# gmarcais/Jellyfish

Measured on AMD Instinct MI355X. Metric: k-mers/sec at k=21 canonical, 150 bp synthetic reads, bit-exact counts, higher is better.
Workload: dtype u64

## Files before the change

### jellyfish_amd/csrc/jfgpu.hip

```cpp
#include <hip/hip_runtime.h>
#include <math.h>
#include <stdint.h>
#include <stdio.h>
#include <string.h>
#include <algorithm>
#include <chrono>
#include <memory>
#include <string>
#include <type_traits>
#include <vector>

#include "../../include/jfgpu.h"
#include "gf2_matrix.hpp"
#include "tuning.hpp"
#include "kernels.hip.hpp"
#include "kernels_part.hip.hpp"
#include "kernels_tile.hip.hpp"
#include "kernels_p1ring.hip.hpp"
#include "kernels_bloom.hip.hpp"
#include "kernels_bloom_part.hip.hpp"
#include "kernels_wide.hip.hpp"
#include "kernels_wide_part.hip.hpp"
#include "kernels_nword.hip.hpp"
#include "kernels_parse.hip.hpp"
// ... 569 lines not shown
  if(!t->part_ok || t->mode == MODE_DIRECT) return false;
  if(t->mode == MODE_PARTITIONED) return true;
  return nbytes >= kPartMinBytes || !t->pending.empty();
}

}

extern "C" {

const char* jfgpu_last_error(void) { return g_err.c_str(); }
int jfgpu_abi_version(void) { return JFGPU_ABI_VERSION; }

int jfgpu_device_count(void) {
  int n = 0;
  if(hipGetDeviceCount(&n) != hipSuccess) return 0;
  return n;
}

int jfgpu_create(const jfgpu_params* p, jfgpu_table** out) {
  if(!p || !out) return fail(JFGPU_E_INVALID, "null argument");
  *out = nullptr;
  if(p->k < 1) return fail(JFGPU_E_INVALID, "mer length must be >= 1");
  if(p->k > 128) return fail(JFGPU_E_UNSUPPORTED, "mer length > 128 (more than four key words) is not built");
  if(p->shard_bits > 8) return fail(JFGPU_E_INVALID, "at most 256 shards");
  if(p->shard_id >= (1u << p->shard_bits)) return fail(JFGPU_E_INVALID, "shard_id out of range");
  int ndev = 0;
  if(hipGetDeviceCount(&ndev) != hipSuccess || ndev == 0)
    return fail(JFGPU_E_NO_DEVICE, "no HIP device: the engine has no CPU fallback");
  int dev = p->device;
  if(dev < 0) HIP_TRY(hipGetDevice(&dev));
  if(dev >= ndev) return fail(JFGPU_E_NO_DEVICE, "device ordinal out of range");
  HIP_TRY(hipSetDevice(dev));

  const bool nword = p->k > 64, wide = p->k > 32 && !nword;
  uint32_t lsize = 0;
  while(lsize < 63 && (1ull << lsize) < p->size) ++lsize;
  if(nword) {
    lsize = std::max(lsize, nword_min_lsize(p->k));
    lsize = std::max<uint32_t>(lsize, kNTileBits + p->shard_bits);
    lsize = std::min<uint32_t>(lsize, 48);
  } else if(wide) {
    lsize = std::max(lsize, wide_min_lsize(p->k));
    lsize = std::max<uint32_t>(lsize, kMaxTileBits + p->shard_bits);
    lsize = std::min<uint32_t>(lsize, 48);
  } else {
    lsize = std::max(lsize, geom_min_lsize(p->k, p->shard_bits));
    lsize = std::max(lsize, p->shard_bits);
    lsize = std::max<uint32_t>(lsize, 1);
    lsize = std::min<uint32_t>(lsize, 2 * p->k);
    if(lsize < p->shard_bits) return fail(JFGPU_E_INVALID, "more shards than 4^k table positions");
  }

  std::unique_ptr<jfgpu_table> t(new jfgpu_table);
  t->tun = Tuning::from_env();
  t->tun.p2_cap = t->tun.p2_cap / kGran * kGran;
  t->params = *p; t->params.matrix_columns = nullptr;
  t->device = dev;
  t->out_counter_len = p->out_counter_len ? p->out_counter_len : 4;
  if(t->out_counter_len > 8) return fail(JFGPU_E_INVALID, "out_counter_len must be <= 8");
  t->wide = wide; t->nword = nword; t->key_words = (2 * p->k + 63) / 64; t->slot_words = nword ? kNWords : wide ? 2 : 1;
  if(nword) {
    if(!nword_geom_init(t->nt.N, p->k, lsize, p->canonical ? 1 : 0, p->shard_bits, p->shard_id)) return fail(JFGPU_E_INVALID, "table geometry does not fit a 256-bit slot");
    t->g = t->nt.N.g;
  } else if(wide) {
    if(!wide_geom_init(t->wt.W, p->k, lsize, p->canonical ? 1 : 0, p->shard_bits, p->shard_id)) return fail(JFGPU_E_INVALID, "table geometry does not fit a 128-bit slot");
    t->g = t->wt.W.g;
  } else if(!geom_init(t->g, p->k, lsize, p->shard_bits, p->shard_id, p->canonical ? 1 : 0, !t->tun.slot64))
    return fail(JFGPU_E_INVALID, "table geometry does not fit a 64-bit slot");

  if(p->matrix_columns) {
    t->matrix.r = lsize; t->matrix.c = 2 * p->k;
    t->matrix.columns.assign(p->matrix_columns, p->matrix_columns + 2 * p->k);
    t->matrix.identity = gf2_is_low_identity(t->matrix);
  } else if(p->matrix_seed) {
    t->matrix = gf2_random(lsize, 2 * p->k, p->matrix_seed);
  } else if(p->k <= 64 && lsize < 2 * p->k && (p->matrix_kind ? p->matrix_kind : (uint32_t)t->tun.matrix) == JFGPU_MATRIX_XORSHIFT) {
    t->xs_matrix = true;
    t->matrix = gf2_xorshift_matrix(lsize, 2 * p->k);
  } else {
    t->ref_matrix = true;
    t->matrix = lsize >= 2 * p->k ? gf2_identity(lsize, 2 * p->k) : gf2_reference_matrix(lsize, 2 * p->k, t->glibc);
  }
  if(!nword) {
    t->g.hash_xs = gf2_is_xorshift(t->matrix) ? 1 : 0;
    if(wide) t->wt.W.g.hash_xs = t->g.hash_xs;
  }
  std::vector<uint64_t> fwd, inv;
  while(!gf2_build_tables(t->matrix, fwd, inv)) {
    if(!t->ref_matrix || t->matrix.identity) return fail(JFGPU_E_INVALID, "hash matrix: low r x r block is singular");
    t->matrix = gf2_reference_matrix(lsize, 2 * p->k, t->glibc);
  }

  hipDeviceProp_t prop;
  HIP_TRY(hipGetDeviceProperties(&prop, dev));
  t->n_cu = prop.multiProcessorCount > 0 ? prop.multiProcessorCount : 256;
  HIP_TRY(hipStreamCreateWithFlags(&t->stream, hipStreamNonBlocking));

  const uint64_t n_slots = 1ull << t->g.lsize_l;
  t->ovf_cap = std::max<uint64_t>(kMinOvf, std::min<uint64_t>(n_slots / 256, 1ull << 26));
  { uint64_t c = 1; while(c < t->ovf_cap) c <<= 1; t->ovf_cap = c; }
  t->returning = t->g.cnt_bits < 40;

  DevTable& d = t->dt;
  d.g = t->g;
  HIP_TRY(hipMalloc((void**)&d.slots, n_slots * slot_bytes_of(t.get())));
  HIP_TRY(hipMalloc((void**)&t->d_fwd, fwd.size() * sizeof(uint64_t)));
  HIP_TRY(hipMalloc((void**)&t->d_inv, inv.size() * sizeof(uint64_t)));
  HIP_TRY(hipMalloc((void**)&d.ovf_key, t->ovf_cap * sizeof(uint64_t)));
  HIP_TRY(hipMalloc((void**)&d.ovf_cnt, t->ovf_cap * sizeof(uint64_t)));
  HIP_TRY(hipMalloc((void**)&d.counters, CTR_COUNT * sizeof(uint64_t)));
  HIP_TRY(hipMalloc((void**)&d.dirty, (size_t)1 << (t->g.lsize_l - t->g.tile_bits)));
  d.fwd_tbl = t->d_fwd; d.inv_tbl = t->d_inv; d.ovf_mask = t->ovf_cap - 1;
  d.max_probe = (uint32_t)std::min<uint64_t>(t->g.tile_mask, 1023);
  HIP_TRY(hipMemcpy(t->d_fwd, fwd.data(), fwd.size() * sizeof(uint64_t), hipMemcpyHostToDevice));
  HIP_TRY(hipMemcpy(t->d_inv, inv.data(), inv.size() * sizeof(uint64_t), hipMemcpyHostToDevice));
  const size_t dump_lds = ((size_t)8 << t->g.tile_bits) + ((size_t)2 << t->g.tile_bits) + (size_t)t->g.nbytes * 2048;
  HIP_TRY(hipFuncSetAttribute((const void*)dump_tiles_kernel, hipFuncAttributeMaxDynamicSharedMemorySize, (int)dump_lds));
  if(nword) {
    NTable& w = t->nt;
    w.slots = d.slots; w.fwd_tbl = d.fwd_tbl; w.inv_tbl = d.inv_tbl; w.ovf_key = d.ovf_key; w.ovf_cnt = d.ovf_cnt;
    w.ovf_mask = d.ovf_mask; w.counters = d.counters; w.max_probe = d.max_probe;
    t->part_ok = false; t->mode = MODE_DIRECT;
    const int nl = (int)(((size_t)32 << kNTileBits) + ((size_t)2 << kNTileBits));
    HIP_TRY(hipFuncSetAttribute((const void*)dump_tiles_words_kernel<NTable>, hipFuncAttributeMaxDynamicSharedMemorySize, nl));
    {
      const int rl = (int)route_lds_bytes(t->g.nbytes, KeyOps<NTable>::kHaloWords);
      HIP_TRY(hipFuncSetAttribute((const void*)route_count_kernel<NTable, false>, hipFuncAttributeMaxDynamicSharedMemorySize, rl));
      HIP_TRY(hipFuncSetAttribute((const void*)route_scatter_kernel<NTable, false>, hipFuncAttributeMaxDynamicSharedMemorySize, rl));
    }
    HIP_TRY(hipFuncSetAttribute((const void*)query_ascii_kernel<NTable>, hipFuncAttributeMaxDynamicSharedMemorySize,
                                (int)query_lds_bytes(t->g.nbytes, KeyOps<NTable>::kHaloWords)));
  } else if(wide) {
    WideTable& w = t->wt;
    w.slots = d.slots; w.fwd_tbl = d.fwd_tbl; w.inv_tbl = d.inv_tbl; w.ovf_key = d.ovf_key; w.ovf_cnt = d.ovf_cnt;
    w.ovf_mask = d.ovf_mask; w.counters = d.counters; w.max_probe = d.max_probe; w.dirty = d.dirty;
    memset(&w.bloom, 0, sizeof w.bloom);
    part_geom_init(t.get());
    const int wl = (int)(((size_t)16 << t->g.tile_bits) + ((size_t)2 << t->g.tile_bits));
    HIP_TRY(hipFuncSetAttribute((const void*)dump_tiles_words_kernel<WideTable>, hipFuncAttributeMaxDynamicSharedMemorySize, wl));
  } else part_geom_init(t.get());
  if(!nword) {
    if(t->tun.mode == 1) t->mode = MODE_DIRECT;
    else if(t->tun.mode == 2 && t->part_ok) t->mode = MODE_PARTITIONED;
  }
  {
#define TATTR2(I, R, S, P, H, M, HL) HIP_TRY(hipFuncSetAttribute((const void*)tile_rank_insert_kernel<I, R, S, P, kTileBlock, H, M, HL>, hipFuncAttributeMaxDynamicSharedMemorySize, (int)tile_rank_lds(sizeof(S), kMaxTileBits, P)))
#define TATTR1(I, R, S, P, H, M) TATTR2(I, R, S, P, H, M, true)
#define TATTR(I, S, P) TATTR1(I, true, S, P, false, false); TATTR1(I, false, S, P, false, false); TATTR1(I, true, S, P, true, false); TATTR1(I, false, S, P, true, false); \
                       TATTR1(I, true, S, P, false, true); TATTR1(I, false, S, P, false, true)
    TATTR(uint32_t, unsigned int, 1); TATTR(uint32_t, unsigned int, 2); TATTR(uint32_t, unsigned long long, 1);
    TATTR(uint64_t, unsigned int, 1); TATTR(uint64_t, unsigned int, 2); TATTR(uint64_t, unsigned long long, 1);
    TATTR2(uint32_t, true, unsigned int, 2, false, false, false); TATTR2(uint32_t, false, unsigned int, 2, false, false, false);
    TATTR2(uint32_t, true, unsigned int, 2, false, true, false); TATTR2(uint32_t, false, unsigned int, 2, false, true, false);
#undef TATTR
#undef TATTR1
#undef TATTR2
    HIP_TRY(hipFuncSetAttribute((const void*)p1_scatter_sorted_kernel<true, true>, hipFuncAttributeMaxDynamicSharedMemorySize, kPTilePos * 6));
    HIP_TRY(hipFuncSetAttribute((const void*)p1_scatter_sorted_kernel<true, false>, hipFuncAttributeMaxDynamicSharedMemorySize, kPTilePos * 6));
    HIP_TRY(hipFuncSetAttribute((const void*)p1_scatter_sorted_kernel<false, true>, hipFuncAttributeMaxDynamicSharedMemorySize, kPTilePos * 6));
    HIP_TRY(hipFuncSetAttribute((const void*)p1_scatter_sorted_kernel<false, false>, hipFuncAttributeMaxDynamicSharedMemorySize, kPTilePos * 6));
#define PATTR(N) HIP_TRY(hipFuncSetAttribute((const void*)p1_keys_scatter_sorted_kernel<N>, hipFuncAttributeMaxDynamicSharedMemorySize, kPTilePos * 6)); \
                 HIP_TRY(hipFuncSetAttribute((const void*)p1_scatter_sorted_kernel<false, false, N>, hipFuncAttributeMaxDynamicSharedMemorySize, kPTilePos * 6))
    PATTR(0); PATTR(6); PATTR(7); PATTR(8);
#undef PATTR
    HIP_TRY(hipFuncSetAttribute((const void*)p1_keys_granule_kernel<true, 0>, hipFuncAttributeMaxDynamicSharedMemorySize, kPTilePos * 6));
    HIP_TRY(hipFuncSetAttribute((const void*)p1_keys_granule_kernel<false, 0>, hipFuncAttributeMaxDynamicSharedMemorySize, kPTilePos * 6));
    HIP_TRY(hipFuncSetAttribute((const void*)p1_keys_granule_kernel<false, 6>, hipFuncAttributeMaxDynamicSharedMemorySize, kPTilePos * 6));
    HIP_TRY(hipFuncSetAttribute((const void*)p1_keys_granule_kernel<false, 7>, hipFuncAttributeMaxDynamicSharedMemorySize, kPTilePos * 6));
    HIP_TRY(hipFuncSetAttribute((const void*)p1_keys_granule_kernel<false, 8>, hipFuncAttributeMaxDynamicSharedMemorySize, kPTilePos * 6));
    {
      const int rl = kGranMaxB * 128 + 128;
#define RATTR(IT, BL, N, CN) HIP_TRY(hipFuncSetAttribute((const void*)p1_ring_kernel<IT, BL, N, CN>, hipFuncAttributeMaxDynamicSharedMemorySize, rl))
      HIP_TRY(hipFuncSetAttribute((const void*)p2_ring_kernel<P2RingDirect>, hipFuncAttributeMaxDynamicSharedMemorySize, rl));
      HIP_TRY(hipFuncSetAttribute((const void*)p2_ring_roles_kernel<uint32_t, 2, P2RingDirect, 1>, hipFuncAttributeMaxDynamicSharedMemorySize, rl));
      HIP_TRY(hipFuncSetAttribute((const void*)p2_ring_roles_kernel<uint32_t, 1, P2RingDirect, 1>, hipFuncAttributeMaxDynamicSharedMemorySize, rl));
      HIP_TRY(hipFuncSetAttribute((const void*)p2_ring_roles_kernel<uint32_t, 2, P2RingDirect, 2>, hipFuncAttributeMaxDynamicSharedMemorySize, rl));
      HIP_TRY(hipFuncSetAttribute((const void*)p2_ring_roles_kernel<uint32_t, 1, P2RingDirect, 2>, hipFuncAttributeMaxDynamicSharedMemorySize, rl));
      HIP_TRY(hipFuncSetAttribute((const void*)p2_ring_roles_kernel<uint32_t, 2, P2RingDirect, 3>, hipFuncAttributeMaxDynamicSharedMemorySize, rl));
      HIP_TRY(hipFuncSetAttribute((const void*)p2_ring_roles_kernel<uint32_t, 1, P2RingDirect, 3>, hipFuncAttributeMaxDynamicSharedMemorySize, rl));
      RATTR(uint32_t, false, 6, 1); RATTR(uint32_t, false, 6, 0); RATTR(uint32_t, true, 0, 2); RATTR(uint32_t, false, 0, 2);
      RATTR(uint32_t, false, kHashXS, 1); RATTR(uint32_t, false, kHashXS, 0); RATTR(uint32_t, false, kHashXSLow, 2);
#undef RATTR
    }
    HIP_TRY(hipFuncSetAttribute((const void*)p2_scatter_sorted_kernel<uint32_t, 16>, hipFuncAttributeMaxDynamicSharedMemorySize, kPBlock * 16 * 4));
    HIP_TRY(hipFuncSetAttribute((const void*)p1_ring_kernel<uint32_t, false, 6, 1, RouteListDirect>, hipFuncAttributeMaxDynamicSharedMemorySize, (int)(kGranMaxB * 128 + 128)));
    HIP_TRY(hipFuncSetAttribute((const void*)p1_ring_kernel<uint32_t, false, 6, 0, RouteListDirect>, hipFuncAttributeMaxDynamicSharedMemorySize, (int)(kGranMaxB * 128 + 128)));
    HIP_TRY(hipFuncSetAttribute((const void*)p1_ring_kernel<uint32_t, false, 0, 2, RouteListDirect>, hipFuncAttributeMaxDynamicSharedMemorySize, (int)(kGranMaxB * 128 + 128)));
    HIP_TRY(hipFuncSetAttribute((const void*)p1_ring_kernel<uint32_t, true, 0, 2, RouteListDirect>, hipFuncAttributeMaxDynamicSharedMemorySize, (int)(kGranMaxB * 128 + 128)));
    HIP_TRY(hipFuncSetAttribute((const void*)p1_ring_kernel<uint32_t, false, kHashXS, 1, RouteListDirect>, hipFuncAttributeMaxDynamicSharedMemorySize, (int)(kGranMaxB * 128 + 128)));
    HIP_TRY(hipFuncSetAttribute((const void*)p1_ring_kernel<uint32_t, false, kHashXS, 0, RouteListDirect>, hipFuncAttributeMaxDynamicSharedMemorySize, (int)(kGranMaxB * 128 + 128)));
    HIP_TRY(hipFuncSetAttribute((const void*)p1_ring_kernel<uint32_t, false, kHashXSLow, 2, RouteListDirect>, hipFuncAttributeMaxDynamicSharedMemorySize, (int)(kGranMaxB * 128 + 128)));
#define SATTR(SW) HIP_TRY(hipFuncSetAttribute((const void*)p2_granule_kernel<uint32_t, TableDirect<true>, kP2PairPer, SW>, hipFuncAttributeMaxDynamicSharedMemorySize, kPBlock * kP2PairPer * 4)); \
                  HIP_TRY(hipFuncSetAttribute((const void*)p2_granule_kernel<uint32_t, TableDirect<false>, kP2PairPer, SW>, hipFuncAttributeMaxDynamicSharedMemorySize, kPBlock * kP2PairPer * 4))
    SATTR(1); SATTR(2); SATTR(4);
#undef SATTR
    HIP_TRY(hipFuncSetAttribute((const void*)p2_granule_kernel<uint64_t, TableDirect<true>, kP2MidPer>, hipFuncAttributeMaxDynamicSharedMemorySize, kPBlock * kP2MidPer * 8));
    HIP_TRY(hipFuncSetAttribute((const void*)p2_granule_kernel<uint64_t, TableDirect<false>, kP2MidPer>, hipFuncAttributeMaxDynamicSharedMemorySize, kPBlock * kP2MidPer * 8));
    HIP_TRY(hipFuncSetAttribute((const void*)p2_granule_kernel<uint32_t, TableDirect<true>, kP2PairPer>, hipFuncAttributeMaxDynamicSharedMemorySize, kPBlock * kP2PairPer * 4));
    HIP_TRY(hipFuncSetAttribute((const void*)p2_granule_kernel<uint32_t, TableDirect<false>, kP2PairPer>, hipFuncAttributeMaxDynamicSharedMemorySize, kPBlock * kP2PairPer * 4));
    HIP_TRY(hipFuncSetAttribute((const void*)p2_scatter_sorted_kernel<uint32_t, kP2PairPer>, hipFuncAttributeMaxDynamicSharedMemorySize, kPBlock * kP2PairPer * 4));
    HIP_TRY(hipFuncSetAttribute((const void*)p2_scatter_sorted_kernel<uint64_t, 14>, hipFuncAttributeMaxDynamicSharedMemorySize, kPBlock * 14 * 8));
    const int gl = kG64Chunk * 10;
    HIP_TRY(hipFuncSetAttribute((const void*)p1_granule64_kernel<true, true, 0>, hipFuncAttributeMaxDynamicSharedMemorySize, gl));
    HIP_TRY(hipFuncSetAttribute((const void*)p1_granule64_kernel<false, true, 0>, hipFuncAttributeMaxDynamicSharedMemorySize, gl));
    HIP_TRY(hipFuncSetAttribute((const void*)p1_granule64_kernel<true, false, 0>, hipFuncAttributeMaxDynamicSharedMemorySize, gl));
    HIP_TRY(hipFuncSetAttribute((const void*)p1_granule64_kernel<false, false, 0>, hipFuncAttributeMaxDynamicSharedMemorySize, gl));
    HIP_TRY(hipFuncSetAttribute((const void*)p1_granule64_kernel<false, false, 7>, hipFuncAttributeMaxDynamicSharedMemorySize, gl));
    HIP_TRY(hipFuncSetAttribute((const void*)p1_granule64_kernel<false, false, 8>, hipFuncAttributeMaxDynamicSharedMemorySize, gl));
    HIP_TRY(hipFuncSetAttribute((const void*)p1_granule64_kernel<false, false, kHashXS>, hipFuncAttributeMaxDynamicSharedMemorySize, gl));
    HIP_TRY(hipFuncSetAttribute((const void*)p1_granule64_kernel<true, false, kHashXS>, hipFuncAttributeMaxDynamicSharedMemorySize, gl));
    HIP_TRY(hipFuncSetAttribute((const void*)p2_granule_kernel<u128, WideDirect<true>, kP2WidePer>, hipFuncAttributeMaxDynamicSharedMemorySize, kPBlock * kP2WidePer * 16));
    HIP_TRY(hipFuncSetAttribute((const void*)p2_granule_kernel<u128, WideDirect<false>, kP2WidePer>, hipFuncAttributeMaxDynamicSharedMemorySize, kPBlock * kP2WidePer * 16));
    HIP_TRY(hipFuncSetAttribute((const void*)p2_scatter_sorted_kernel<u128, 7>, hipFuncAttributeMaxDynamicSharedMemorySize, kPBlock * 7 * 16));
    const int wl = kWideChunk * 18 + 16 * 2048, wt = 16 << kMaxTileBits;
    HIP_TRY(hipFuncSetAttribute((const void*)p1_wide_granule_kernel<true, true>, hipFuncAttributeMaxDynamicSharedMemorySize, wl));
    HIP_TRY(hipFuncSetAttribute((const void*)p1_wide_granule_kernel<true, false>, hipFuncAttributeMaxDynamicSharedMemorySize, wl));
    HIP_TRY(hipFuncSetAttribute((const void*)p1_wide_granule_kernel<false, true>, hipFuncAttributeMaxDynamicSharedMemorySize, wl));
    HIP_TRY(hipFuncSetAttribute((const void*)p1_wide_granule_kernel<false, false>, hipFuncAttributeMaxDynamicSharedMemorySize, wl));
    HIP_TRY(hipFuncSetAttribute((const void*)p1_wide_granule_kernel<true, false, true>, hipFuncAttributeMaxDynamicSharedMemorySize, wl));
    HIP_TRY(hipFuncSetAttribute((const void*)p1_wide_granule_kernel<false, false, true>, hipFuncAttributeMaxDynamicSharedMemorySize, wl));
    HIP_TRY(hipFuncSetAttribute((const void*)tile_insert_wide_kernel<true>, hipFuncAttributeMaxDynamicSharedMemorySize, wt));
    HIP_TRY(hipFuncSetAttribute((const void*)tile_insert_wide_kernel<false>, hipFuncAttributeMaxDynamicSharedMemorySize, wt));
    HIP_TRY(hipFuncSetAttribute((const void*)tile_insert_wide_pipe_kernel<true>, hipFuncAttributeMaxDynamicSharedMemorySize, wt));
    HIP_TRY(hipFuncSetAttribute((const void*)tile_insert_wide_pipe_kernel<false>, hipFuncAttributeMaxDynamicSharedMemorySize, wt));
  }
  jfgpu_table* raw = t.release();
  int rc = jfgpu_clear(raw);
  if(rc) { jfgpu_destroy(raw); return rc; }
  *out = raw;
  return JFGPU_OK;
}

void jfgpu_destroy(jfgpu_table* t) {
  if(!t) return;
  hipSetDevice(t->device);
  if(t->stream) hipStreamSynchronize(t->stream);
  prof_collect(t);
  for(auto e : t->ev_pool) hipEventDestroy(e);
  hipFree(t->dt.slots); hipFree(t->d_fwd); hipFree(t->d_inv);
  if(t->d_dt) hipFree(t->d_dt);
  hipFree(t->dt.ovf_key); hipFree(t->dt.ovf_cnt); hipFree(t->dt.counters); hipFree(t->dt.dirty);
  for(int i = 0; i < 2; ++i) { if(t->d_stage[i]) hipFree(t->d_stage[i]); if(t->stage_done[i]) hipEventDestroy(t->stage_done[i]); }
  if(t->d_dump) hipFree(t->d_dump);
  if(t->d_bcache) hipFree(t->d_bcache);
  if(t->d_tile_off) hipFree(t->d_tile_off);
  part_discard(t);
  if(t->d_M1) hipFree(t->d_M1);
  if(t->d_strag) hipFree(t->d_strag);
  if(t->d_strag2) hipFree(t->d_strag2);
  if(t->d_strag2_n) hipFree(t->d_strag2_n);
  if(t->d_strag_n) hipFree(t->d_strag_n);
  if(t->d_M2) hipFree(t->d_M2);
  if(t->ws) hipFree(t->ws);
  if(t->stream2) hipStreamDestroy(t->stream2);
  for(auto ev : t->flush_ev) if(ev) hipEventDestroy(ev);
  if(t->flush_done) hipEventDestroy(t->flush_done);
  if(t->stream) hipStreamDestroy(t->stream);
  delete t;
}

int jfgpu_get_info(const jfgpu_table* t, jfgpu_info* o) {
  if(!t || !o) return fail(JFGPU_E_INVALID, "null argument");
  memset(o, 0, sizeof(*o));
  o->k = t->g.k; o->key_len = t->g.key_bits; o->canonical = t->g.canonical;
  o->lsize = t->g.lsize_g; o->size = 1ull << t->g.lsize_g; o->local_size = 1ull << t->g.lsize_l;
  o->shard_bits = t->g.shard_bits; o->shard_id = t->g.shard_id;
  o->val_len = t->g.cnt_bits; o->slot_bytes = (uint32_t)slot_bytes_of(t); o->tile_slots = 1u << t->g.tile_bits;
  o->matrix_identity = t->matrix.identity ? 1 : 0;
  o->out_counter_len = t->out_counter_len;
  o->max_reprobe = t->dt.max_probe;
  o->table_bytes = (1ull << t->g.lsize_l) * slot_bytes_of(t);
  return JFGPU_OK;
}

int jfgpu_get_matrix(const jfgpu_table* t, uint64_t* columns) {
  if(!t || !columns) return fail(JFGPU_E_INVALID, "null argument");
  memcpy(columns, t->matrix.columns.data(), sizeof(uint64_t) * t->matrix.c);
  return JFGPU_OK;
}

int jfgpu_clear(jfgpu_table* t) {
  if(t) { t->failed = 0; t->failed_msg.clear(); }
  int rc = use(t); if(rc) return rc;
  part_discard(t);
  HIP_TRY(hipMemsetAsync(t->dt.slots, 0, (1ull << t->g.lsize_l) * slot_bytes_of(t), t->stream));
  HIP_TRY(hipMemsetAsync(t->dt.ovf_key, 0, t->ovf_cap * sizeof(uint64_t), t->stream));
  HIP_TRY(hipMemsetAsync(t->dt.ovf_cnt, 0, t->ovf_cap * sizeof(uint64_t), t->stream));
  HIP_TRY(hipMemsetAsync(t->dt.counters, 0, CTR_COUNT * sizeof(uint64_t), t->stream));
  HIP_TRY(hipMemsetAsync(t->dt.dirty, 0, (size_t)1 << (t->g.lsize_l - t->g.tile_bits), t->stream));
  HIP_TRY(hipStreamSynchronize(t->stream));
  t->pristine = true; t->occ_known = 0; t->fed_since = 0; t->direct_seen = 0; t->occ_bound = 0; t->bigval_bound = 0; t->ovf_failed_need = 0;
  t->flushes_plain = 0; t->flushes_heavy = 0;
  t->n_p2_roles = t->n_p2_ring = t->n_p2_sort = t->n_p2_exact = t->n_p1_ring = t->n_p1_other = t->n_tile_dense = 0;
  return JFGPU_OK;
}

int jfgpu_sync(jfgpu_table* t) {
  int rc = use(t); if(rc) return rc;
  rc = part_flush(t); if(rc) return rc;
  HIP_TRY(hipStreamSynchronize(t->stream));
#ifdef JFGPU_PHASE_PROF
  { unsigned long long c[24], z[24] = {0};
    if(hipMemcpyFromSymbol(c, HIP_SYMBOL(g_phase_prof), sizeof c) == hipSuccess) {
      fprintf(stderr, "[phase prof] P1 (ring): stage %llu  encode+hash+append %llu  (barrier) %llu  units out %llu  finish %llu\n",
              c[0], c[1], c[2], c[3], c[4]);
      fprintf(stderr, "[phase prof] P2: (barrier) %llu  load %llu  hist %llu  scan %llu  lds-scatter %llu  write-out %llu  finish %llu\n",
// ... 552 lines not shown
```

### jellyfish_amd/csrc/kernels_tile.hip.hpp

```cpp
#pragma once
#include "kernels_part.hip.hpp"

namespace jfgpu {

__device__ __attribute__((noinline)) void ovf_add_call(uint64_t* ovf_key, uint64_t* ovf_cnt, uint64_t ovf_mask, uint64_t* counters,
                                                       uint64_t slot, uint64_t units) {
  DevTable V; V.ovf_key = ovf_key; V.ovf_cnt = ovf_cnt; V.ovf_mask = ovf_mask; V.counters = counters;
  ovf_add(V, slot, units);
}

__device__ __forceinline__ uint32_t wg_uniform(uint32_t v) {
#if defined(__HIP_DEVICE_COMPILE__) && !defined(JFGPU_EMU)
  return (uint32_t)__builtin_amdgcn_readfirstlane((int)v);
#else
  return v;
#endif
}

__device__ __forceinline__ void lds_wait_all() {
#if defined(__HIP_DEVICE_COMPILE__) && !defined(JFGPU_EMU)
  __builtin_amdgcn_s_waitcnt(0xC07F);
#endif
}

#ifndef JFGPU_T_BLOCK
#define JFGPU_T_BLOCK 512
#endif
constexpr int kTileBlock = JFGPU_T_BLOCK;
constexpr uint32_t kQueueLook = 2;
#ifndef JFGPU_T_QUEUE
#define JFGPU_T_QUEUE 6144
#endif
constexpr uint32_t kTileQueueBytes = JFGPU_T_QUEUE;

constexpr size_t tile_rank_hdr(size_t nslots) { return (nslots >> kBucketBits) * 2 + 16; }
inline size_t tile_rank_lds(size_t slot_bytes, uint32_t tile_bits, int tpb) {
  const size_t nslots = (size_t)tpb << tile_bits;
  return tile_rank_hdr(nslots) + nslots * slot_bytes + kTileQueueBytes;
}

template <typename ITEM, bool RETURNING, typename SLOT, int TPB, int BLOCK = kTileBlock, bool HEAVY = false, bool SAMPLE = false, bool HOLES = true>
__global__ __launch_bounds__(BLOCK, (BLOCK >= 512 ? 2 * BLOCK / 256 : 4)) void tile_rank_insert_kernel(DevTable T, SegList S, uint64_t tile0, uint32_t n_tiles) {
  constexpr int NP = ((sizeof(ITEM) == 8 || (BLOCK < 512 && TPB == 1)) ? 4608 : 9216) / BLOCK;
  constexpr uint32_t kVec = 16 / sizeof(SLOT);
  constexpr uint32_t kB = 1u << kBucketBits;
  constexpr uint32_t kBV = kB / kVec;
  constexpr uint32_t kSlotBits = 8 * sizeof(SLOT);
  JF_DYN_LDS(s_raw);
  const TableGeom& g = T.g;
  constexpr uint32_t tsz = 1u << kMaxTileBits, nslots = TPB * tsz, nbkt = nslots >> kBucketBits, tmask = tsz - 1;
  constexpr uint32_t NBK = nbkt / BLOCK;
  static_assert(HOLES || (!HEAVY && sizeof(ITEM) == 4), "the hole-free instantiation is the plain kernel's, for 4-byte items");
  constexpr uint32_t kHdr = (uint32_t)tile_rank_hdr(nslots);
  uint32_t* const s_cnt = reinterpret_cast<uint32_t*>(s_raw);
  SLOT* const s_tile = reinterpret_cast<SLOT*>(s_raw + kHdr);
  constexpr uint32_t qcap = kTileQueueBytes / sizeof(ITEM) / (BLOCK / 64);
  static_assert(qcap >= 64, "phase C stages one held-back item per lane through the queue");
  ITEM* const s_q = reinterpret_cast<ITEM*>(s_raw + kHdr + (size_t)nslots * sizeof(SLOT)) + (threadIdx.x >> 6) * qcap;
  SLOT* const gslots = reinterpret_cast<SLOT*>(T.slots);
  const SLOT lmask = (SLOT)g.low_mask, inc = (SLOT)g.inc, occ = (SLOT)g.occ_bit;
  const uint32_t cshift = g.tag_bits + 1, idshift = kSlotBits - cshift;
  const uint32_t lane = threadIdx.x & 63;
  const unsigned long long below = lane ? (~0ull >> (64 - lane)) : 0ull;
  const ITEM hole = (ITEM)~(ITEM)0;

  auto unit_dirty = [&](uint32_t t) -> uint32_t {
    if(TPB == 2) return *reinterpret_cast<const uint16_t*>(T.dirty + tile0 + 2 * (uint64_t)t);
    return T.dirty[tile0 + t];
  };
  auto zero_counters = [&]() {
    for(uint32_t i = threadIdx.x; i < (nbkt >> 1); i += BLOCK) s_cnt[i] = 0;
  };
  auto zero_tile = [&]() {
    for(uint32_t i = threadIdx.x * kVec; i < nslots; i += BLOCK * kVec) *reinterpret_cast<uint4*>(s_tile + i) = make_uint4(0, 0, 0, 0);
  };
  auto load_tile = [&](const SLOT* gt, uint32_t d) {
    for(uint32_t b = threadIdx.x; b < nbkt; b += BLOCK) {
      const bool ld = (d >> (8 * ((b << kBucketBits) >> kMaxTileBits))) & 0xFFu;
      uint32_t c = 0;
#pragma unroll
      for(uint32_t q = 0; q < kBV; ++q) {
        uint4 v = make_uint4(0, 0, 0, 0);
        if(ld) v = *reinterpret_cast<const uint4*>(gt + ((size_t)b << kBucketBits) + q * kVec);
        *reinterpret_cast<uint4*>(s_tile + ((size_t)b << kBucketBits) + q * kVec) = v;
        if(sizeof(SLOT) == 4) c += (v.x != 0) + (v.y != 0) + (v.z != 0) + (v.w != 0);
        else c += ((v.x | v.y) != 0) + ((v.z | v.w) != 0);
      }
      reinterpret_cast<uint16_t*>(s_cnt)[b] = (uint16_t)c;
    }
  };
  auto home_of = [&](ITEM x) -> uint32_t {
    if constexpr(sizeof(ITEM) == 4) return ((uint32_t)x >> g.rem_bits) & (nslots - 1);
    else return (uint32_t)((uint64_t)x >> g.rem_bits) & (nslots - 1);
  };
  auto load_bucket = [&](uint32_t bs, SLOT (&w)[kB]) {
#pragma unroll
    for(uint32_t q = 0; q < kBV; ++q) {
      const uint4 v = *reinterpret_cast<const uint4*>(s_tile + bs + q * kVec);
      if constexpr(sizeof(SLOT) == 4) { w[4 * q] = (SLOT)v.x; w[4 * q + 1] = (SLOT)v.y; w[4 * q + 2] = (SLOT)v.z; w[4 * q + 3] = (SLOT)v.w; }
      else { w[2 * q] = (SLOT)(((uint64_t)v.y << 32) | v.x); w[2 * q + 1] = (SLOT)(((uint64_t)v.w << 32) | v.z); }
    }
  };
  auto store_bucket = [&](uint32_t bs, const SLOT (&w)[kB]) {
#pragma unroll
    for(uint32_t q = 0; q < kBV; ++q) {
      uint4 v;
      if constexpr(sizeof(SLOT) == 4) v = make_uint4((uint32_t)w[4 * q], (uint32_t)w[4 * q + 1], (uint32_t)w[4 * q + 2], (uint32_t)w[4 * q + 3]);
      else v = make_uint4((uint32_t)w[2 * q], (uint32_t)((uint64_t)w[2 * q] >> 32), (uint32_t)w[2 * q + 1], (uint32_t)((uint64_t)w[2 * q + 1] >> 32));
      *reinterpret_cast<uint4*>(s_tile + bs + q * kVec) = v;
    }
  };
  auto has_dups = [&](const SLOT (&w)[kB]) -> bool {
    SLOT sh[kB];
#pragma unroll
    for(uint32_t i = 0; i < kB; ++i) sh[i] = w[i] << idshift;
    bool d = false;
#pragma unroll
    for(uint32_t j = 1; j < kB; ++j) {
      bool e = false;
#pragma unroll
      for(uint32_t i = 0; i < j; ++i) e = e | (sh[i] == sh[j]);
      d = d | (e & (w[j] != 0));
    }
    return d;
  };
  auto merge_bucket = [&](SLOT (&w)[kB], uint64_t bucket_slot0) {
    const SLOT cmask = (SLOT)g.cnt_max;
    SLOT carry[kB];
#pragma unroll
    for(uint32_t i = 0; i < kB; ++i) carry[i] = 0;
#pragma unroll
    for(uint32_t j = 1; j < kB; ++j)
#pragma unroll
      for(uint32_t i = 0; i < j; ++i) {
        const bool same = (w[j] != 0) & (w[i] != 0) & (((w[i] ^ w[j]) & lmask) == 0);
        const SLOT sum = (SLOT)(w[i] >> cshift) + (same ? (SLOT)(w[j] >> cshift) : (SLOT)0);
        w[i] = (w[i] & lmask) | (SLOT)((sum & cmask) << cshift);
        carry[i] += (SLOT)(sum >> g.cnt_bits);
        w[j] = same ? (SLOT)0 : w[j];
      }
    SLOT o[kB], oc[kB];
#pragma unroll
    for(uint32_t i = 0; i < kB; ++i) { o[i] = 0; oc[i] = 0; }
    uint32_t n = 0;
#pragma unroll
    for(uint32_t j = 0; j < kB; ++j) {
      const bool ne = w[j] != 0;
#pragma unroll
      for(uint32_t d = 0; d <= j; ++d) { const bool here = ne & (n == d); o[d] = here ? w[j] : o[d]; oc[d] = here ? carry[j] : oc[d]; }
      n += ne ? 1u : 0u;
    }
    SLOT any = 0;
#pragma unroll
    for(uint32_t q = 0; q < kB; ++q) { w[q] = o[q]; any |= oc[q]; }
    if(RETURNING && any != 0) {
#pragma unroll
      for(uint32_t q = 0; q < kB; ++q) if(oc[q]) ovf_add_call(T.ovf_key, T.ovf_cnt, T.ovf_mask, T.counters, bucket_slot0 + q, (uint64_t)oc[q]);
    }
  };
  auto merge_tile = [&](uint64_t unit_slot0) {
    constexpr uint32_t MB0 = (TPB == 2 && sizeof(ITEM) + sizeof(SLOT) == 8 && NBK >= 4) ? 4 : (NBK >= 2 ? 2 : 1);
    constexpr uint32_t Rmax = nbkt / (BLOCK / 64);
    static_assert(Rmax >= 128, "the merge list must fit the bucket counters");
    constexpr uint32_t R = Rmax >= 512 ? 512 : Rmax >= 256 ? 256 : 128;
    constexpr uint32_t MBr = R >= 512 ? 4 : R >= 256 ? 2 : 1;
    constexpr uint32_t MBw = 16 / kB >= 1 ? 16 / kB : 1;
    constexpr uint32_t MB = MB0 < MBr ? (MB0 < MBw ? MB0 : MBw) : (MBr < MBw ? MBr : MBw);
    static_assert((BLOCK / 64) * R * 2 <= nbkt * 2, "the merge list must fit the bucket counters");
    uint16_t* const lst = reinterpret_cast<uint16_t*>(s_cnt) + (threadIdx.x >> 6) * R;
    uint32_t head = 0, cnt = 0;
#pragma unroll 1
    for(uint32_t k0 = 0; k0 < NBK; k0 += MB) {
      SLOT wb[MB][kB];
#pragma unroll
      for(uint32_t k = 0; k < MB; ++k) load_bucket((threadIdx.x + (k0 + k) * BLOCK) << kBucketBits, wb[k]);
#pragma unroll
      for(uint32_t k = 0; k < MB; ++k) {
        const bool dup = has_dups(wb[k]);
        const unsigned long long m = __ballot(dup);
        if(dup) lst[(head + cnt + (uint32_t)__popcll(m & below)) & (R - 1)] = (uint16_t)(threadIdx.x + (k0 + k) * BLOCK);
        cnt += (uint32_t)__popcll(m);
      }
      const bool last = k0 + MB >= NBK;
      while(cnt >= 64 || (last && cnt)) {
        const uint32_t n = cnt < 64 ? cnt : 64;
        (void)__ballot(true);
        if(lane < n) {
          const uint32_t b = lst[(head + lane) & (R - 1)];
          SLOT w[kB];
          load_bucket(b << kBucketBits, w);
          merge_bucket(w, unit_slot0 + ((uint64_t)b << kBucketBits));
          store_bucket(b << kBucketBits, w);
        }
        head += n; cnt -= n;
      }
    }
  };
  auto store_tile = [&](SLOT* gt, uint32_t t) {
#pragma unroll
    for(uint32_t k = 0; k < NBK; ++k) {
      const uint32_t b = threadIdx.x + k * BLOCK;
#pragma unroll
      for(uint32_t q = 0; q < kBV; ++q) {
        const uint4 v = *reinterpret_cast<const uint4*>(s_tile + ((size_t)b << kBucketBits) + q * kVec);
        *reinterpret_cast<uint4*>(gt + ((size_t)b << kBucketBits) + q * kVec) = v;
        *reinterpret_cast<uint4*>(s_tile + ((size_t)b << kBucketBits) + q * kVec) = make_uint4(0, 0, 0, 0);
      }
    }
    zero_counters();
    if(threadIdx.x == 0) {
      if(TPB == 2) *reinterpret_cast<uint16_t*>(T.dirty + tile0 + 2 * (uint64_t)t) = 0x0101;
      else T.dirty[tile0 + t] = 1;
    }
  };
  auto slow_insert = [&](ITEM x, uint64_t unit_slot0) {
    constexpr uint32_t LK = kQueueLook;
    const SLOT low = occ | (SLOT)((uint64_t)x & (g.occ_bit - 1)), neww = inc | low;
    const uint32_t h = home_of(x), hbase = h & ~tmask, hb = h & tmask & ~(kB - 1u);
    const uint32_t max_steps = (T.max_probe >> kBucketBits) + 1;
    for(uint32_t step = 0; step < max_steps; ) {
      SLOT w[LK][kB];
#pragma unroll
      for(uint32_t k = 0; k < LK; ++k) load_bucket(hbase + ((hb + ((step + k) << kBucketBits)) & tmask), w[k]);
      uint32_t hitm = 0, empm = 0;
#pragma unroll
      for(uint32_t k = 0; k < LK; ++k)
#pragma unroll
        for(uint32_t i = 0; i < kB; ++i) {
          hitm |= (uint32_t)((w[k][i] & lmask) == low) << (kB * k + i);
          empm |= (uint32_t)(w[k][i] == 0) << (kB * k + i);
        }
      for(uint32_t cand = hitm | empm; cand; cand &= cand - 1) {
        const uint32_t j = (uint32_t)__ffs((int)cand) - 1u;
        if(step + (j >> kBucketBits) >= max_steps) { step = max_steps; break; }
        const uint32_t at = hbase + ((hb + (step << kBucketBits) + j) & tmask);
        bool add = (hitm >> j) & 1;
        if(!add) {
          const SLOT was = atomicCAS(&s_tile[at], (SLOT)0, neww);
          if(was == 0) return;
          add = (was & lmask) == low;
        }
        if(add) {
          if(RETURNING) {
            const SLOT prev = atomicAdd(&s_tile[at], inc);
            if(((uint64_t)prev >> cshift) + 1 > g.cnt_max) ovf_add_call(T.ovf_key, T.ovf_cnt, T.ovf_mask, T.counters, unit_slot0 + at, 1);
          } else atomicAdd(&s_tile[at], inc);
          return;
        }
      }
      step += LK;
    }
    atomicAdd((unsigned long long*)&T.counters[CTR_FULL], 1ull);
  };

  [[maybe_unused]] PhaseClk pc;
  auto rank_request = [&](const ITEM (&it)[NP], uint32_t vm, uint32_t (&old)[NP]) {
#pragma unroll
    for(int r = 0; r < NP; ++r)
      if((vm >> r) & 1) { const uint32_t b = home_of(it[r]) >> kBucketBits; old[r] = atomicAdd(&s_cnt[b >> 1], 1u << ((b & 1) * 16)); }
  };
  auto rank_request_dense = [&](const ITEM (&it)[NP], uint32_t nf, ITEM tail, bool tv, uint32_t (&old)[NP], uint32_t& told) {
#pragma unroll
    for(int r = 0; r < NP; ++r)
      if((uint32_t)r < nf) { const uint32_t b = home_of(it[r]) >> kBucketBits; old[r] = atomicAdd(&s_cnt[b >> 1], 1u << ((b & 1) * 16)); }
    if(tv) { const uint32_t b = home_of(tail) >> kBucketBits; told = atomicAdd(&s_cnt[b >> 1], 1u << ((b & 1) * 16)); }
  };
  [[maybe_unused]] uint32_t smp_items = 0, smp_queued = 0;
  auto place_round = [&](ITEM (&it)[NP], uint32_t vm, const uint32_t (&old)[NP], uint64_t unit_slot0, const ITEM* again, auto&& after_a,
                         [[maybe_unused]] ITEM tail = 0, [[maybe_unused]] uint32_t told = 0, [[maybe_unused]] bool tv = false) {
    uint32_t qn = 0, pend = 0;
    [[maybe_unused]] uint32_t ovm = 0;
#pragma unroll
    for(int r = 0; r < NP; ++r) JF_OPAQUE(it[r]);
    auto place_item = [&](ITEM x, uint32_t o, bool valid, uint32_t bit) {
      bool ov = false;
      if(valid) {
        const uint32_t b = home_of(x) >> kBucketBits;
        const uint32_t rank = (o >> ((b & 1) * 16)) & 0xFFFFu;
        if(rank < kB) s_tile[(b << kBucketBits) + rank] = inc | occ | (SLOT)((uint64_t)x & (g.occ_bit - 1));
        else ov = true;
      }
      if constexpr(HEAVY) { if(ov) ovm |= 1u << bit; }
      else {
        const unsigned long long m = __ballot(ov);
        if(ov) {
          const uint32_t at = qn + (uint32_t)__popcll(m & below);
          if(at < qcap) s_q[at] = x; else pend |= 1u << bit;
        }
        qn += (uint32_t)__popcll(m);
      }
    };
    if constexpr(HOLES) {
#pragma unroll
      for(int r = 0; r < NP; ++r) place_item(it[r], old[r], (vm >> r) & 1, (uint32_t)r);
      if constexpr(SAMPLE) smp_items += (uint32_t)__popc(vm);
    } else {
      lds_wait_all();
#pragma unroll
      for(int r = 0; r < NP; ++r)
        if((uint32_t)r < vm) place_item(it[r], old[r], true, (uint32_t)r);
      JF_OPAQUE(tail);
      place_item(tail, told, tv, (uint32_t)NP);
      if constexpr(SAMPLE) smp_items += vm + (tv ? 1u : 0u);
    }
    if constexpr(SAMPLE) smp_queued += qn;
    if constexpr(!HEAVY) after_a();
    lds_barrier();
    JF_PHASE(pc, 2);
    merge_tile(unit_slot0);
    lds_barrier();
    JF_PHASE(pc, 6);
    uint32_t nq = qn < qcap ? qn : qcap;
    if constexpr(HEAVY) {
      uint32_t q2 = 0, carry = 0;
      constexpr int CB = kB == 4 ? 6 : 3;
#pragma unroll
      for(int r0 = 0; r0 < NP; r0 += CB) {
        SLOT wb[CB][kB];
#pragma unroll
        for(int k = 0; k < CB; ++k)
          if(r0 + k < NP && ((ovm >> (r0 + k)) & 1)) load_bucket(home_of(it[r0 + k < NP ? r0 + k : 0]) & ~(kB - 1u), wb[k]);
#pragma unroll
        for(int k = 0; k < CB; ++k) {
          if(r0 + k >= NP) continue;
          const int r = r0 + k;
          bool miss = false;
          if((ovm >> r) & 1) {
            const ITEM x = it[r];
            const SLOT low = occ | (SLOT)((uint64_t)x & (g.occ_bit - 1));
            const uint32_t bs = home_of(x) & ~(kB - 1u);
            int hit = -1;
#pragma unroll
            for(int i = (int)kB - 1; i >= 0; --i) if((wb[k][i] & lmask) == low) hit = i;
            if(hit >= 0) {
              if(RETURNING) {
                const SLOT prev = atomicAdd(&s_tile[bs + hit], inc);
                if(((uint64_t)prev >> cshift) + 1 > g.cnt_max) carry |= 1u << r;
              } else atomicAdd(&s_tile[bs + hit], inc);
            } else miss = true;
          }
          const unsigned long long m2 = __ballot(miss);
          if(miss) {
            const uint32_t at = q2 + (uint32_t)__popcll(m2 & below);
            if(at < qcap) s_q[at] = it[r]; else pend |= 1u << r;
          }
          q2 += (uint32_t)__popcll(m2);
        }
      }
      (void)__ballot(true);
      after_a();
      while(carry) {
        const uint32_t r = (uint32_t)__ffs((int)carry) - 1u; carry &= carry - 1;
        const ITEM x = again[r * BLOCK + threadIdx.x];
        const SLOT low = occ | (SLOT)((uint64_t)x & (g.occ_bit - 1));
        const uint32_t bs = home_of(x) & ~(kB - 1u);
        SLOT w[kB];
        load_bucket(bs, w);
        uint32_t hit = 0;
#pragma unroll
        for(int i = (int)kB - 1; i >= 1; --i) if((w[i] & lmask) == low) hit = (uint32_t)i;
        if((w[0] & lmask) == low) hit = 0;
        ovf_add_call(T.ovf_key, T.ovf_cnt, T.ovf_mask, T.counters, unit_slot0 + bs + hit, 1);
      }
      nq = q2 < qcap ? q2 : qcap;
    }
    for(;;) {
      for(uint32_t i = lane; i < nq; i += 64) slow_insert(s_q[i], unit_slot0);
      const unsigned long long m = __ballot(pend != 0);
      if(!m) break;
      if(pend) {
        uint32_t r = (uint32_t)__ffs((int)pend) - 1u;
        pend &= pend - 1;
        if constexpr(!HOLES) { if(r == (uint32_t)NP) r = vm; }
        s_q[(uint32_t)__popcll(m & below)] = again[r * BLOCK + threadIdx.x];
      }
      nq = (uint32_t)__popcll(m);
      (void)__ballot(true);
    }
    JF_PHASE(pc, 5);
    lds_barrier();
    JF_PHASE(pc, 3);
  };
  zero_counters();
  zero_tile();
  lds_barrier();
  const uint64_t* off = S.off[0];
  const uint32_t sh = S.sh[0];
  const bool holes = sh != 0;
  static_assert(NP < 32, "a round's items and the partial row are bits of one word");
  const ITEM* src = reinterpret_cast<const ITEM*>(S.items[0]);
  const uint32_t G = gridDim.x;
  constexpr uint64_t kRound = (uint64_t)NP * BLOCK;
  uint32_t t = blockIdx.x;
  uint64_t a0 = 0, b0 = 0, a1 = 0, b1 = 0; uint32_t d0 = 0, d1 = 0;
  ITEM cur[NP];
  [[maybe_unused]] ITEM tail = 0;
  auto fetch = [&](uint64_t a, uint64_t b) {
    const ITEM* ub = src + a;
    const uint32_t n = (uint32_t)((b - a) < kRound ? (b - a) : kRound);
    if(b <= a) return;
    uint32_t tid = threadIdx.x;
    JF_OPAQUE(tid);
    if constexpr(!HOLES) {
      const uint32_t nf = wg_uniform(n / BLOCK);
#pragma unroll
      for(int r = 0; r < NP; ++r)
        if((uint32_t)r < nf) cur[r] = ub[(uint32_t)r * BLOCK + tid];
      const uint32_t i = nf * BLOCK + tid;
      tail = ub[i < n ? i : n - 1];
      return;
    }
#pragma unroll
    for(int r = 0; r < NP; ++r) {
      const uint32_t i = (uint32_t)r * BLOCK + tid;
      cur[r] = ub[i < n ? i : n - 1];
    }
  };
  if(t < n_tiles) { a0 = off[(size_t)t << sh]; b0 = off[((size_t)t << sh) + 1]; d0 = unit_dirty(t); }
  if(t + G < n_tiles) { a1 = off[(size_t)(t + G) << sh]; b1 = off[((size_t)(t + G) << sh) + 1]; d1 = unit_dirty(t + G); }
  fetch(a0, b0);
  uint64_t c0 = a0;
  while(t < n_tiles) {
    if(b0 <= a0) {
      uint64_t a2 = 0, b2 = 0; uint32_t d2 = 0;
      if(t + 2 * G < n_tiles) { a2 = off[(size_t)(t + 2 * G) << sh]; b2 = off[((size_t)(t + 2 * G) << sh) + 1]; d2 = unit_dirty(t + 2 * G); }
      t += G; a0 = a1; b0 = b1; d0 = d1; a1 = a2; b1 = b2; d1 = d2; c0 = a0;
      fetch(a0, b0);
      continue;
    }
    const bool first = c0 == a0, last = c0 + kRound >= b0;
    const uint64_t unit_slot0 = (tile0 + (uint64_t)TPB * t) << kMaxTileBits;
    SLOT* gt = gslots + unit_slot0;
    JF_PHASE(pc, 0);
    const uint32_t n0 = (uint32_t)((b0 - c0) < kRound ? (b0 - c0) : kRound);
    uint32_t vm = 0, tid = threadIdx.x;
    JF_OPAQUE(tid);
    [[maybe_unused]] bool tv = false;
    if constexpr(HOLES) {
#pragma unroll
      for(int r = 0; r < NP; ++r)
        if((uint32_t)r * BLOCK + tid < n0 && !(holes && cur[r] == hole)) vm |= 1u << r;
    } else {
      vm = wg_uniform(n0 / BLOCK);
      tv = vm * BLOCK + tid < n0;
    }
    const uint32_t d_eff = first ? d0 : (TPB == 2 ? 0x0101u : 1u);
    if(d_eff) { load_tile(gt, d_eff); lds_barrier(); }
    uint32_t old[NP];
    [[maybe_unused]] uint32_t told = 0;
    if constexpr(HOLES) rank_request(cur, vm, old);
    else rank_request_dense(cur, vm, tail, tv, old, told);
    JF_PHASE(pc, 1);
    uint64_t a2 = 0, b2 = 0; uint32_t d2 = 0;
    if(last && t + 2 * G < n_tiles) { a2 = off[(size_t)(t + 2 * G) << sh]; b2 = off[((size_t)(t + 2 * G) << sh) + 1]; d2 = unit_dirty(t + 2 * G); }
    if constexpr(HOLES) place_round(cur, vm, old, unit_slot0, src + c0, [&] { if(last) fetch(a1, b1); else fetch(c0 + kRound, b0); });
    else place_round(cur, vm, old, unit_slot0, src + c0, [&] { if(last) fetch(a1, b1); else fetch(c0 + kRound, b0); }, tail, told, tv);
    store_tile(gt, t);
    lds_barrier();
    JF_PHASE(pc, 4);
    if(last) { t += G; a0 = a1; b0 = b1; d0 = d1; a1 = a2; b1 = b2; d1 = d2; c0 = a0; }
    else c0 += kRound;
  }
  JF_PHASE_FLUSH(pc, 16);
  if constexpr(SAMPLE) {
    uint32_t w = smp_items;
    for(int o = 32; o > 0; o >>= 1) w += __shfl_down(w, o, 64);
    if(lane == 0) {
      atomicAdd((unsigned long long*)&T.counters[CTR_T_ITEMS], (unsigned long long)w);
      atomicAdd((unsigned long long*)&T.counters[CTR_T_QUEUED], (unsigned long long)smp_queued);
    }
  }
}

}
```

Measured before the change: 15.82 billion.

## Streamline dense tile rank/place path with raw LDS addressing and deferred overflow queueing

In the dense (non-HOLES) tile insert path, bucket rank requests and slot stores now go through raw LDS address-space pointers computed with alignbit/bfe, replacing the home_of/shift arithmetic. Per-item overflow ballots during placement are removed. Overflowing items are instead re-read from the source and handed off to the queue after the merge barrier, in up to four rounds per thread. The aim is fewer VALU ops and wave-wide ballots in the hot placement loop. In exchange it assumes a zero static-LDS base (checked on the host), and any thread with more than four overflows is pushed to the pending path.

```diff
diff --git a/jellyfish_amd/csrc/jfgpu.hip b/jellyfish_amd/csrc/jfgpu.hip
--- a/jellyfish_amd/csrc/jfgpu.hip
+++ b/jellyfish_amd/csrc/jfgpu.hip
@@ -745,6 +745,13 @@
     TATTR(uint64_t, unsigned int, 1); TATTR(uint64_t, unsigned int, 2); TATTR(uint64_t, unsigned long long, 1);
     TATTR2(uint32_t, true, unsigned int, 2, false, false, false); TATTR2(uint32_t, false, unsigned int, 2, false, false, false);
     TATTR2(uint32_t, true, unsigned int, 2, false, true, false); TATTR2(uint32_t, false, unsigned int, 2, false, true, false);
+#if !defined(JFGPU_EMU)
+#define TBASE0(R, M) do { hipFuncAttributes fa_; \
+      HIP_TRY(hipFuncGetAttributes(&fa_, (const void*)tile_rank_insert_kernel<uint32_t, R, unsigned int, 2, kTileBlock, false, M, false>)); \
+      if(fa_.sharedSizeBytes != 0) return fail(JFGPU_E_HIP, "tile_rank_insert_kernel: static LDS in front of the tile (JF_LDS_AT)"); } while(0)
+    TBASE0(true, false); TBASE0(false, false); TBASE0(true, true); TBASE0(false, true);
+#undef TBASE0
+#endif
 #undef TATTR
 #undef TATTR1
 #undef TATTR2
diff --git a/jellyfish_amd/csrc/kernels_tile.hip.hpp b/jellyfish_amd/csrc/kernels_tile.hip.hpp
--- a/jellyfish_amd/csrc/kernels_tile.hip.hpp
+++ b/jellyfish_amd/csrc/kernels_tile.hip.hpp
@@ -20,6 +20,38 @@
 __device__ __forceinline__ void lds_wait_all() {
 #if defined(__HIP_DEVICE_COMPILE__) && !defined(JFGPU_EMU)
   __builtin_amdgcn_s_waitcnt(0xC07F);
+#endif
+}
+
+__device__ __forceinline__ uint32_t rotr32(uint32_t x, uint32_t s) {
+#if defined(__HIP_DEVICE_COMPILE__) && !defined(JFGPU_EMU)
+  return __builtin_amdgcn_alignbit(x, x, s);
+#else
+  s &= 31u;
+  return s ? (x >> s) | (x << (32u - s)) : x;
+#endif
+}
+
+__device__ __forceinline__ uint32_t bfe_u32(uint32_t x, uint32_t off, uint32_t width) {
+#if defined(__HIP_DEVICE_COMPILE__) && !defined(JFGPU_EMU)
+  return __builtin_amdgcn_ubfe(x, off, width);
+#else
+  return (x >> (off & 31u)) & ((1u << width) - 1u);
+#endif
+}
+
+#if defined(__HIP_DEVICE_COMPILE__) && !defined(JFGPU_EMU)
+#define JF_LDS_PTR(type) __attribute__((address_space(3))) type*
+#define JF_LDS_AT(type, raw, off) (reinterpret_cast<JF_LDS_PTR(type)>((uint32_t)(off)))
+#else
+#define JF_LDS_PTR(type) type*
+#define JF_LDS_AT(type, raw, off) (reinterpret_cast<type*>((raw) + (off)))
+#endif
+__device__ __forceinline__ uint32_t lds_fetch_add(JF_LDS_PTR(uint32_t) p, uint32_t v) {
+#if defined(__HIP_DEVICE_COMPILE__) && !defined(JFGPU_EMU)
+  return __hip_atomic_fetch_add(p, v, __ATOMIC_RELAXED, __HIP_MEMORY_SCOPE_AGENT);
+#else
+  return atomicAdd(p, v);
 #endif
 }
 
@@ -259,19 +291,42 @@
     for(int r = 0; r < NP; ++r)
       if((vm >> r) & 1) { const uint32_t b = home_of(it[r]) >> kBucketBits; old[r] = atomicAdd(&s_cnt[b >> 1], 1u << ((b & 1) * 16)); }
   };
+  [[maybe_unused]] const uint32_t cw_shift = g.rem_bits + kBucketBits - 1, odd_bit = g.rem_bits + kBucketBits;
+  [[maybe_unused]] auto rank_add = [&](ITEM x) -> uint32_t {
+    const uint32_t w = ((uint32_t)x >> cw_shift) & (((nbkt >> 1) - 1u) << 2);
+    return lds_fetch_add(JF_LDS_AT(uint32_t, s_raw, w), bfe_u32((uint32_t)x, odd_bit, 1) * 0xFFFFu + 1u);
+  };
   auto rank_request_dense = [&](const ITEM (&it)[NP], uint32_t nf, ITEM tail, bool tv, uint32_t (&old)[NP], uint32_t& told) {
 #pragma unroll
     for(int r = 0; r < NP; ++r)
-      if((uint32_t)r < nf) { const uint32_t b = home_of(it[r]) >> kBucketBits; old[r] = atomicAdd(&s_cnt[b >> 1], 1u << ((b & 1) * 16)); }
-    if(tv) { const uint32_t b = home_of(tail) >> kBucketBits; told = atomicAdd(&s_cnt[b >> 1], 1u << ((b & 1) * 16)); }
+      if((uint32_t)r < nf) old[r] = rank_add(it[r]);
+    if(tv) told = rank_add(tail);
   };
   [[maybe_unused]] uint32_t smp_items = 0, smp_queued = 0;
+  [[maybe_unused]] uint32_t smp_over = 0;
+  constexpr int kHand = 4;
   auto place_round = [&](ITEM (&it)[NP], uint32_t vm, const uint32_t (&old)[NP], uint64_t unit_slot0, const ITEM* again, auto&& after_a,
                          [[maybe_unused]] ITEM tail = 0, [[maybe_unused]] uint32_t told = 0, [[maybe_unused]] bool tv = false) {
     uint32_t qn = 0, pend = 0;
     [[maybe_unused]] uint32_t ovm = 0;
 #pragma unroll
     for(int r = 0; r < NP; ++r) JF_OPAQUE(it[r]);
+    [[maybe_unused]] ITEM qx[kHand];
+    [[maybe_unused]] auto hand_off = [&]() {
+      uint32_t rest = ovm;
+#pragma unroll
+      for(int j = 0; j < kHand; ++j) {
+        const unsigned long long m = __ballot(rest != 0);
+        if(!m) break;
+        if(rest) {
+          const uint32_t at = qn + (uint32_t)__popcll(m & below);
+          if(at < qcap) s_q[at] = qx[j]; else pend |= rest & (0u - rest);
+        }
+        rest &= rest - 1u;
+        qn += (uint32_t)__popcll(m);
+      }
+      pend |= rest;
+    };
     auto place_item = [&](ITEM x, uint32_t o, bool valid, uint32_t bit) {
       bool ov = false;
       if(valid) {
@@ -296,20 +351,51 @@
       if constexpr(SAMPLE) smp_items += (uint32_t)__popc(vm);
     } else {
       lds_wait_all();
+      static_assert(HOLES || (kBucketBits == 2 && sizeof(SLOT) == 4 && sizeof(ITEM) == 4), "place_dense: buckets of four 4-byte slots, 4-byte items");
+      const uint32_t hrot = (g.rem_bits + 32u - kBucketBits) & 31u, low_m = (uint32_t)(g.occ_bit - 1);
+      uint32_t top = (uint32_t)(inc | occ);
+      JF_OPAQUE(top);
+      uint32_t okm = ~((1u << vm) - 1u) & ~((tv ? 1u : 0u) << NP);
+      auto place_dense = [&](ITEM x, uint32_t o, uint32_t bit, bool valid) {
+        const uint32_t h = rotr32((uint32_t)x, hrot);
+        const uint32_t rank = bfe_u32(o, h & 16u, 16);
+        if(valid && rank < kB) {
+          *JF_LDS_AT(uint32_t, s_raw, kHdr + (h & ((nslots - kB) << 2)) + (rank << 2)) = ((uint32_t)x & low_m) | top;
+          okm |= 1u << bit;
+        }
+      };
 #pragma unroll
       for(int r = 0; r < NP; ++r)
-        if((uint32_t)r < vm) place_item(it[r], old[r], true, (uint32_t)r);
+        if((uint32_t)r < vm) place_dense(it[r], old[r], (uint32_t)r, true);
       JF_OPAQUE(tail);
-      place_item(tail, told, tv, (uint32_t)NP);
-      if constexpr(SAMPLE) smp_items += vm + (tv ? 1u : 0u);
-    }
-    if constexpr(SAMPLE) smp_queued += qn;
-    if constexpr(!HEAVY) after_a();
+      place_dense(tail, told, (uint32_t)NP, tv);
+      ovm = ~okm;
+      if constexpr(SAMPLE) { smp_items += vm + (tv ? 1u : 0u); smp_over += (uint32_t)__popc(ovm); }
+      uint32_t tid = threadIdx.x, rest = ovm;
+      JF_OPAQUE(tid);
+#pragma unroll
+      for(int j = 0; j < kHand; ++j) {
+        qx[j] = 0;
+        if(rest) {
+          uint32_t r = (uint32_t)__ffs((int)rest) - 1u;
+          if(r == (uint32_t)NP) r = vm;
+          qx[j] = again[r * BLOCK + tid];
+        }
+        rest &= rest - 1u;
+      }
+    }
+    if constexpr(SAMPLE && HOLES) smp_queued += qn;
+    if constexpr(!HEAVY && HOLES) after_a();
     lds_barrier();
     JF_PHASE(pc, 2);
     merge_tile(unit_slot0);
     lds_barrier();
     JF_PHASE(pc, 6);
+    if constexpr(!HOLES) {
+      hand_off();
+      (void)__ballot(true);
+      after_a();
+    }
     uint32_t nq = qn < qcap ? qn : qcap;
     if constexpr(HEAVY) {
       uint32_t q2 = 0, carry = 0;
@@ -465,6 +551,11 @@
   if constexpr(SAMPLE) {
     uint32_t w = smp_items;
     for(int o = 32; o > 0; o >>= 1) w += __shfl_down(w, o, 64);
+    if constexpr(!HOLES) {
+      uint32_t q = smp_over;
+      for(int o = 32; o > 0; o >>= 1) q += __shfl_down(q, o, 64);
+      smp_queued = q;
+    }
     if(lane == 0) {
       atomicAdd((unsigned long long*)&T.counters[CTR_T_ITEMS], (unsigned long long)w);
       atomicAdd((unsigned long long*)&T.counters[CTR_T_QUEUED], (unsigned long long)smp_queued);
```

After: 15.57 billion. 0.984x the previous value.
